# gkv856/speaker_embedding_GE2E_loss

Hardware: AMD Instinct MI355X
Metric: GE2E loss+backward throughput, (spk x utt) batches/sec at N=64 M=10 D=256 (higher is better)
Workload: dtype f32; 1 GPU; cfg2: N=64 M=10 D=256 softmax GE2E fwd+bwd, B=16384 batches per launch per GPU, w=10 b=-5; mode=loss, N=64, M=10, D=256, variant=softmax, batches_per_launch=16384, impl=team, parallelism=dp1 (whole batches per rank, no data-path collective)

## Files before the change

speaker_embedding_ge2e_loss_amd/csrc/ge2e_team_fwd.hip:

```cpp
#include <algorithm>

#include "ge2e_common.hpp"
#include "ge2e_split_gemm.hpp"
#include "ge2e_team.hpp"
#include "ge2e_team_kernel.hpp"
#include "ge2e_team_dev.hpp"

namespace ge2e {

size_t team_fwd_lds_bytes(int rt, int D) {
    return (size_t)2 * rt * D * 2 + (size_t)2 * rt * XP * 4 + (size_t)(2 * rt * 4 + 32 + 16) * sizeof(float);
}

template <int NCH, int MR, int RBT, bool CONTRAST>
__global__ __launch_bounds__(512, 2) void ge2e_team_fwd_kernel(Problem p, TeamKWs L, FusedWs F) {
    extern __shared__ __attribute__((aligned(16))) float smem_f[];
    constexpr int D = 64 * NCH;
    constexpr int P = D;
    const int DG = RBT ? D : p.D;
    const unsigned ROWBG = (unsigned)DG * 4u;
    constexpr TeamKX XO = team_exchange(D);
    constexpr unsigned SC4 = XO.cst[0];
    constexpr int RBC = RBT ? RBT : RBMAX;
    const int RB = RBT ? RBT : L.rt / 16;
    const int RT = 16 * RB;
    const int RBr = RB;
    constexpr bool CT_X = RBT != 0;
    _Float16* const ETh = reinterpret_cast<_Float16*>(smem_f);
    _Float16* const ETl = ETh + RT * P;
    float* const XB0 = reinterpret_cast<float*>(ETl + RT * P);
    float* const XB1 = XB0 + RT * XP;
    float* const RS = XB1 + RT * XP;
    float* const RED = RS + 2 * RT * 4;
    int* const SH = reinterpret_cast<int*>(RED + 32);

    constexpr bool MEX = RBT != 0;
    const int N = MEX ? 64 : p.N, M = MEX ? MR : p.M, NM = N * M;
    const int tid = threadIdx.x;
    const int lane = tid & 63;
    const int wid = __builtin_amdgcn_readfirstlane(tid >> 6);

    TeamCtl* const ctl = reinterpret_cast<TeamCtl*>(p.ws);
    TeamKFlags* const flags = reinterpret_cast<TeamKFlags*>(ctl + 1);
    const TeamId id = team_form(ctl, SH, team_launch_id(p.launch_seq));
    if (id.team == -2) {
        team_redo<NCH>(p, L, F, smem_f, (int)gridDim.x, (int)blockIdx.x);
        __syncthreads();
        if (blockIdx.x == 0 && tid < 64) team_untrusted_done(ctl, (int)(L.head_bytes / 16), team_launch_id(p.launch_seq));
        return;
    }
    if (id.nct == 0 && blockIdx.x == 0 && tid == 0)
        __hip_atomic_store(&ctl->abort_, 1u, __ATOMIC_RELAXED, __HIP_MEMORY_SCOPE_AGENT);
    bool gave_up = id.nct == 0;
    [&]() __attribute__((always_inline)) {
    if (id.team < 0) return;
    TeamKFlags* const fl = flags + id.team;
    const __amdgpu_buffer_rsrc_t rsX = make_rsrc(
        reinterpret_cast<const char*>(p.ws) + L.head_bytes + (size_t)id.team * XO.stride, XO.stride);

    const int spm = MEX ? 8 : L.spm;
    const int w_bits = __builtin_amdgcn_readfirstlane(__float_as_int(p.w ? *p.w : p.w_imm));
    const int b_bits = __builtin_amdgcn_readfirstlane(__float_as_int(p.b ? *p.b : p.b_imm));
    const float eps = p.eps, eps_cos = p.eps_cos;
#define GE2E_TF_CONSTS()                                                                       \
    int wb_ = w_bits, bb_ = b_bits, mc_ = M, le_ = __float_as_int(p.log_eps);                  \
    asm volatile("" : "+s"(wb_), "+s"(bb_), "+s"(mc_), "+s"(le_));                             \
    const float w = __int_as_float(wb_), bias = __int_as_float(bb_);                           \
    const float eps_cos2 = eps_cos * eps_cos;                                                  \
    const float fM = (float)mc_, inv_m = rcp_nr(fM), inv_m1 = rcp_nr((float)(mc_ - 1));       \
    (void)w; (void)bias; (void)eps_cos2; (void)fM; (void)inv_m; (void)inv_m1; (void)le_
    constexpr float LOG2E = 1.4426950408889634f, LN2 = 0.6931471805599453f;

    for (int i = tid; i < RT * P / 8; i += 512) {
        reinterpret_cast<float4*>(ETh)[i] = zero4();
        reinterpret_cast<float4*>(ETl)[i] = zero4();
    }
    for (int i = tid; i < 2 * RT; i += 512) reinterpret_cast<float4*>(RS)[i] = zero4();
    __syncthreads();

    float4 ra[MR], rb2[MR];
    float sn_cur = 0.f, ss_cur = 0.f, sn_prev = 0.f, ss_prev = 0.f;
#define GE2E_TF_LOAD_ROWS(REG, BI)                                                                       \
    do {                                                                                                 \
        int lq_ = lane;                                                                                  \
        asm volatile("" : "+v"(lq_));                                                                    \
        const unsigned vrow_ = 4 * lq_ < DG ? (unsigned)lq_ * 16u : OOB;                                 \
        const bool on_ = has_spk && (BI) < p.B;                                                          \
        const __amdgpu_buffer_rsrc_t rs_ = make_rsrc(p.E + (size_t)(on_ ? (BI) : 0) * NM * DG, (unsigned)NM * ROWBG); \
        _Pragma("unroll") for (int i = 0; i < MR; ++i)                                                   \
            REG[i] = bload4<GE2E_T2_E_AUX>(rs_, (on_ && i < M) ? vrow_ : OOB, (unsigned)(j * M + min(i, M - 1)) * ROWBG); \
    } while (0)
#ifdef GE2E_TF_WITH_PRIO
#define GE2E_TF_PRIO(n) __builtin_amdgcn_s_setprio(n)
#else
#define GE2E_TF_PRIO(n)
#endif
#define GE2E_TF_LOADR_SETUP(BI)                                                                          \
    int lq_ = lane;                                                                                      \
    asm volatile("" : "+v"(lq_));                                                                        \
    const unsigned vrow_ = 4 * lq_ < DG ? (unsigned)lq_ * 16u : OOB;                                     \
    const bool on_ = has_spk && (BI) < p.B;                                                              \
    const __amdgpu_buffer_rsrc_t rs_ = make_rsrc(p.E + (size_t)(on_ ? (BI) : 0) * NM * DG, (unsigned)NM * ROWBG)
#define GE2E_TF_LOADR(REG, I_)                                                                           \
    do {                                                                                                 \
        if ((I_) < MR) {                                                                                 \
            __builtin_amdgcn_sched_barrier(0);                                                           \
            REG[(I_) < MR ? (I_) : 0] = bload4<GE2E_T2_E_AUX>(rs_, (on_ && (I_) < M) ? vrow_ : OOB,      \
                                                              (unsigned)(j * M + min((I_), M - 1)) * ROWBG); \
            __builtin_amdgcn_sched_barrier(0);                                                           \
        }                                                                                                \
    } while (0)
#define GE2E_TF_LANE()                                                  \
    int lv_ = lane;                                                     \
    asm volatile("" : "+v"(lv_));                                       \
    const int l15 = lv_ & 15, q = lv_ >> 4, d4 = 4 * lv_;               \
    const bool dact = D == 256 || d4 < D;                               \
    (void)l15; (void)q; (void)d4; (void)dact

    GE2E_PROF_DECL(20)
    {
        const int j0 = id.member * spm;
        const int my_spm = MEX ? 8 : max(0, min(spm, N - j0));
        const bool has_spk = wid < my_spm;
        const int j = j0 + wid;
        GE2E_TF_LOAD_ROWS(ra, id.team);
        GE2E_TF_LOAD_ROWS(rb2, id.team + id.nct);
    }
    const TeamId id_outer = id;
    bool failed = false;
    int nsig = 0;
    const int wid_outer = wid, member_outer = id.member, tid_outer = tid, m_outer = M;
    float4 sc_pend = zero4();
    int sc_batch = -1;
    auto sc_flush = [&]() __attribute__((always_inline)) {
        if (sc_batch >= 0) {
            const float l = oct_sum(sc_pend.x), a = oct_sum(sc_pend.y), c = oct_sum(sc_pend.z);
            if ((threadIdx.x & 63) == 0) {
                if (p.loss) p.loss[sc_batch] = l;
                if (p.dw) p.dw[sc_batch] = a;
                if (p.db) p.db[sc_batch] = c;
            }
            sc_batch = -1;
        }
    };
    const int nb = id.team < p.B ? (p.B - id.team + id.nct - 1) / id.nct : 0;
    int seq = 0;
    auto body = [&](float4 (&R0)[MR]) __attribute__((always_inline)) {
        int wid_o = wid_outer, mem_o = member_outer, tid_o = tid_outer, m_o = m_outer;
        asm volatile("" : "+s"(wid_o), "+s"(mem_o), "+v"(tid_o), "+s"(m_o));
        const int wid = wid_o, tid = tid_o, lane = tid & 63, M = MEX ? MR : m_o, NM = N * M;
        TeamId id = id_outer;
        id.member = mem_o;
        const int j0 = id.member * spm;
        const int my_spm = MEX ? 8 : max(0, min(spm, N - j0));
        const bool has_spk = wid < my_spm;
        const int j = j0 + wid;
        const int kslot = 8 * id.member + wid;
        const int rbase = wid * M;
        const int tX = wid & 3, khX = wid >> 2;
        const int bi = id.team + seq * id.nct;
        const bool have_cur = seq < nb, have_prev = seq > 0;
        const int buf = seq & 1, pbuf = buf ^ 1;
        sn_prev = sn_cur; ss_prev = ss_cur;

        h8 xa[NCH][2];
        int lx_ = lane;
        asm volatile("" : "+v"(lx_));
        const unsigned oa = have_prev ? XO.chr[pbuf] + ((unsigned)tX * (4u * NCH) + (unsigned)khX * NCH) * 1024u + (unsigned)lx_ * 16u : OOB;
#define GE2E_TF_XA_LOAD(K_)                                                                                        \
    do {                                                                                                           \
        if ((K_) < 2 * NCH) {                                                                                      \
            __builtin_amdgcn_sched_barrier(0);                                                                     \
            xa[((K_) < 2 * NCH ? (K_) : 0) >> 1][(K_) & 1] =                                                       \
                bload_h8<AUX_L2>(rsX, oa + 1024u * (unsigned)((K_) >> 1) + (((K_) & 1) ? 2048u * NCH : 0u), 0);    \
            __builtin_amdgcn_sched_barrier(0);                                                                     \
        }                                                                                                          \
    } while (0)
        if (!have_cur) static_for<0, 2 * NCH>([&](auto kc) { GE2E_TF_XA_LOAD(decltype(kc)::value); });
        if (have_cur) {
            GE2E_TF_LANE();
            GE2E_TF_CONSTS();
            float4 s = zero4();
            static_for<0, MR>([&](auto ic) {
                constexpr int i = decltype(ic)::value;
                if (i < M) { s.x += R0[i].x; s.y += R0[i].y; s.z += R0[i].z; s.w += R0[i].w; }
                GE2E_TF_XA_LOAD(i);
            });
            const float4 c = scale4(s, inv_m);
            float sqs[2] = {dot4(c, c), dot4(s, s)};
            wave_sum_to_sgpr<2>(sqs);
            float rn, kap, nc;
            unit_stats_bf(sqs[0], eps_cos, eps_cos2, rn, kap, nc);
            if (!has_spk) { rn = 0.f; nc = 0.f; }
            sn_cur = has_spk ? fM * nc : 0.f;
            ss_cur = has_spk ? sqs[1] : 0.f;
            h4 hi, lo;
            split4_scaled(c, rn * kSplitScale, hi, lo);
            const unsigned blk = (unsigned)(kslot >> 4) * (4u * NCH) + (unsigned)(lv_ >> 3);
            const unsigned vh = dact ? blk * 1024u + (unsigned)(((lv_ >> 1) & 3) * 16 + (kslot & 15)) * 16u + (unsigned)(lv_ & 1) * 8u : OOB;
            __builtin_amdgcn_raw_buffer_store_b64(__builtin_bit_cast(u32x2, hi), rsX, vh + XO.chr[buf], 0, 0);
            __builtin_amdgcn_raw_buffer_store_b64(__builtin_bit_cast(u32x2, lo), rsX, vh + XO.chr[buf] + 2048u * NCH, 0, 0);
        }
        GE2E_PROF(0);
        GE2E_TF_PRIO(1);

        auto phase_x = [&]() __attribute__((always_inline)) {
        if (have_prev) {
            GE2E_TF_LANE();
            float* const XBk = khX ? XB1 : XB0;
            const int fx = (4 * (l15 & 3) + ((4 - (l15 >> 2)) & 3)) & ((D % 128 == 0) ? 15 : 7);
            h8 fb[2][2];
            f32x4 acc[2] = {acc_zero4(), acc_zero4()};
            int xs[NCH];
#pragma unroll
            for (int s2 = 0; s2 < NCH; ++s2) xs[s2] = l15 * P + (((4 * (khX * NCH + s2) + q) ^ fx) << 3);
#define TF_X_LOAD(T_)                                                                                     \
    do {                                                                                                  \
        const _Float16* const pp_ = ETh + xs[(T_) % NCH] + 16 * ((T_) / NCH) * P;                         \
        fb[(T_) & 1][0] = frag_row(pp_);                                                                  \
        fb[(T_) & 1][1] = frag_row(pp_ + RT * P);                                                         \
    } while (0)
#define TF_X_STORE(RB_)                                                                       \
    *reinterpret_cast<float4*>(XBk + (16 * (RB_) + l15) * XP + 16 * tX + 4 * q) =             \
        make_float4(acc[(RB_) & 1][0], acc[(RB_) & 1][1], acc[(RB_) & 1][2], acc[(RB_) & 1][3])
            TF_X_LOAD(0);
#pragma unroll
            for (int rb = 0; rb < RBC; ++rb) {
                if (CT_X || rb < RBr) {
                    acc[rb & 1] = acc_zero4();
#pragma unroll
                    for (int s = 0; s < NCH; ++s) {
                        const int t = rb * NCH + s;
                        if (t + 1 < RBC * NCH && (CT_X || t + 1 < RBr * NCH)) TF_X_LOAD(t + 1);
                        mfma16x3(acc[rb & 1], xa[s][0], xa[s][1], fb[t & 1][0], fb[t & 1][1]);
                        __builtin_amdgcn_sched_barrier(0);
                    }
                    if (rb > 0) { TF_X_STORE(rb - 1); }
                }
            }
            if (CT_X) { TF_X_STORE(RBT - 1); }
            else {
#pragma unroll
                for (int rb = 0; rb < RBC; ++rb)
                    if (rb == RBr - 1) { TF_X_STORE(rb); }
            }
#undef TF_X_LOAD
#undef TF_X_STORE
        }
        };
        phase_x();
        sc_flush();
        GE2E_PROF(1);

        asm volatile("s_waitcnt vmcnt(0)" ::: "memory");
        GE2E_PROF(2);
        __syncthreads();
        if (tid == 0) add_agent(&fl->c1, 1u);
        ++nsig;
        GE2E_PROF(3);
        GE2E_TF_PRIO(3);

        h4 hiv[MR], lov[MR];
        auto phase_a2c = [&]() __attribute__((always_inline)) {
        if (have_cur && has_spk) {
            GE2E_TF_LANE();
            GE2E_TF_CONSTS();
            float eev[MR];
#pragma unroll
            for (int i = 0; i < MR; ++i) eev[i] = i < M ? dot4(R0[i], R0[i]) : 0.f;
            const float ee_l = wave_sums_scatter<MR>(eev, lv_);
            float rne_l, ke_l, ne_l;
            unit_stats_bf(ee_l, eps_cos, eps_cos2, rne_l, ke_l, ne_l);
            {
                const int rho = lv_ >> 4, irow = 4 * (lv_ & 15) + (((rho & 1) << 1) | (rho >> 1));
                if ((lv_ & 15) < (MR + 3) / 4 && irow < M)
                    *reinterpret_cast<float4*>(RS + (buf * RT + rbase + irow) * 4) = make_float4(rne_l, ke_l, ee_l, ne_l);
            }
            const float rs_l = rne_l * kSplitScale;
            float scv[MR];
#pragma unroll
            for (int i = 0; i < MR; ++i) scv[i] = lane_get(rs_l, scatter_lane(i));
#pragma unroll
            for (int i = 0; i < MR; ++i)
                if (i < M) split4_scaled_hi_u(R0[i], scv[i], hiv[i]);
#pragma unroll
            for (int i = 0; i < MR; ++i)
                if (i < M) split4_scaled_lo_u(R0[i], scv[i], hiv[i], lov[i]);
        }
        };
        phase_a2c();
        if (have_cur && has_spk) {
            GE2E_TF_LANE();
#pragma unroll
            for (int i = 0; i < MR; ++i)
                if (i < M && dact) {
                    const int eo = et_off<D>(rbase + i, d4);
                    *reinterpret_cast<h4*>(ETh + eo) = hiv[i];
                    *reinterpret_cast<h4*>(ETl + eo) = lov[i];
                }
        }
        const bool spread_loads = have_prev && has_spk;
        if (!spread_loads) GE2E_TF_LOAD_ROWS(R0, bi + 2 * id.nct);
        GE2E_PROF(4);
        GE2E_TF_PRIO(1);

        float loss_acc = 0.f, dw_acc = 0.f, db_acc = 0.f;
        if (have_prev && has_spk) {
            GE2E_TF_LANE();
            GE2E_TF_CONSTS();
            const float w2 = w * LOG2E, b2 = (w * eps + bias) * LOG2E, leps2 = __int_as_float(le_) * LOG2E;
            const int rr = lv_ >> 2, qq = lv_ & 3;
            const bool rv = rr < M;
            const int r = rbase + min(rr, M - 1);
            const int ko = kslot;
            const int sb = (ko & ~3) + 16 * qq;
            const int jo = ko & 3;
            const bool own_lane = qq == 0;
            const bool all_valid = N == NC;
            const bool want_wb = p.dw != nullptr || p.db != nullptr;
            GE2E_TF_LOADR_SETUP(bi + 2 * id.nct);
            float x[16];
            float4 xa4[4], xb4[4];
#pragma unroll
            for (int jj = 0; jj < 4; ++jj) {
                const int s4 = (sb + 4 * jj) & (NC - 1);
                xa4[jj] = *reinterpret_cast<const float4*>(XB0 + r * XP + s4);
                xb4[jj] = *reinterpret_cast<const float4*>(XB1 + r * XP + s4);
            }
            GE2E_TF_LOADR(R0, 0);
#pragma unroll
            for (int jj = 0; jj < 4; ++jj) {
                const float4 a = xa4[jj], b = xb4[jj];
                x[4 * jj + 0] = a.x + b.x; x[4 * jj + 1] = a.y + b.y; x[4 * jj + 2] = a.z + b.z; x[4 * jj + 3] = a.w + b.w;
                if (jj == 1) GE2E_TF_LOADR(R0, 1);
            }
            GE2E_TF_LOADR(R0, 2);
            const float xo = (XB0[r * XP + ko] + XB1[r * XP + ko]) * kSplitInv2;
            const float4 rs0 = *reinterpret_cast<const float4*>(RS + (pbuf * RT + r) * 4);
            const float rne = rs0.x, ee = rs0.z, ne = rs0.w;
            const float es = xo * sn_prev * ne;
            const float eu = (es - ee) * inv_m1;
            const float uu = fmaxf((ss_prev - 2.0f * es + ee) * (inv_m1 * inv_m1), 0.0f);
            float rnu, ku, nu;
            unit_stats_bf(uu, eps_cos, eps_cos2, rnu, ku, nu);
            const float cosd = eu * rne * rnu;
            GE2E_TF_LOADR(R0, 3);
            const float sjj2 = fmaf(w2, cosd, b2);
            const float w2s = w2 * kSplitInv2;
            auto vld = [&](int jx) {
                const int s = (sb + jx) & (NC - 1);
                return all_valid || (s & 7) < max(0, min(spm, N - (s >> 3) * spm));
            };
            bool ownj[4];
#pragma unroll
            for (int jx = 0; jx < 4; ++jx) ownj[jx] = own_lane && jo == jx;
            float per, coefsum = 0.f, db_row = 0.f;
            GE2E_TF_PRIO(0);
            GE2E_TF_LOADR(R0, 4);
            if (!CONTRAST) {
                float xm0 = ownj[0] ? x[1] : x[0], xm1 = ownj[1] ? x[0] : x[1], xm2 = ownj[2] ? x[3] : x[2], xm3 = ownj[3] ? x[2] : x[3];
                float xm;
                if (w2 >= 0.f) {
                    xm = fmaxf(fmaxf(xm0, xm1), fmaxf(xm2, xm3));
#pragma unroll
                    for (int jx = 4; jx < 16; jx += 2) xm = fmaxf(fmaxf(x[jx], x[jx + 1]), xm);
                } else {
                    xm = fminf(fminf(xm0, xm1), fminf(xm2, xm3));
#pragma unroll
                    for (int jx = 4; jx < 16; jx += 2) xm = fminf(fminf(x[jx], x[jx + 1]), xm);
                }
                GE2E_TF_LOADR(R0, 5);
                float mx = quad_max(fmaf(w2s, xm, b2));
                mx = fmaxf(fmaxf(mx, sjj2), leps2);
                const float t = b2 - mx;
                float gv[16];
#pragma unroll
                for (int jx = 0; jx < 16; ++jx) {
                    gv[jx] = __builtin_amdgcn_exp2f(fmaf(w2s, x[jx], t));
                    if ((jx & 3) == 3) GE2E_TF_LOADR(R0, 6 + (jx >> 2));
                }
                static_for<10, MR>([&](auto ic) { GE2E_TF_LOADR(R0, decltype(ic)::value); });
                if (!all_valid) {
#pragma unroll
                    for (int jx = 0; jx < 16; ++jx) gv[jx] = vld(jx) ? gv[jx] : 0.f;
                }
#pragma unroll
                for (int jx = 0; jx < 4; ++jx) gv[jx] = ownj[jx] ? 0.f : gv[jx];
                float z4[4] = {gv[0], gv[1], gv[2], gv[3]}, a4[4] = {0.f, 0.f, 0.f, 0.f};
#pragma unroll
                for (int jx = 4; jx < 16; ++jx) z4[jx & 3] += gv[jx];
                const float zl = (z4[0] + z4[1]) + (z4[2] + z4[3]);
                float al = 0.f;
                if (want_wb) {
#pragma unroll
                    for (int jx = 0; jx < 16; ++jx) a4[jx & 3] = fmaf(gv[jx], x[jx], a4[jx & 3]);
                    al = (a4[0] + a4[1]) + (a4[2] + a4[3]);
                }
                const float zp = quad_sum(zl);
                const float zoff = zp + __builtin_amdgcn_exp2f(leps2 - mx);
                const float z = zoff + __builtin_amdgcn_exp2f(sjj2 - mx);
                per = LN2 * ((mx - sjj2) + __builtin_amdgcn_logf(z));
                if (want_wb) {
                    const float ap = quad_sum(al);
                    const float rz = rcp_nr(z);
                    const float ad0 = -zoff * rz;
                    coefsum = fmaf(ap * kSplitInv2, rz, ad0 * cosd);
                    db_row = fmaf(zp, rz, ad0);
                }
            } else {
                static_for<5, MR>([&](auto ic) { GE2E_TF_LOADR(R0, decltype(ic)::value); });
                float best = -INFINITY, bx = 0.f; int besti = 0x7fffffff;
#pragma unroll
                for (int jx = 0; jx < 16; ++jx) {
                    const int s = (sb + jx) & (NC - 1);
                    const bool ok = vld(jx) && !(jx < 4 && ownj[jx & 3]);
                    const float sve = ok ? fmaf(w2s, x[jx], b2) : -INFINITY;
                    if (ok && (sve > best || (sve == best && s < besti))) { best = sve; besti = s; bx = x[jx]; }
                }
                const int loci = besti;
                quad_argmax(best, besti);
                bx = quad_sum(loci == besti && besti != 0x7fffffff ? bx : 0.f);
                const float pos = rcp_nr(1.0f + __builtin_amdgcn_exp2f(-sjj2));
                const float neg = (N > 1) ? rcp_nr(1.0f + __builtin_amdgcn_exp2f(-best)) : 0.0f;
                per = 1.0f - pos + neg;
                const float ad0 = -pos * (1.0f - pos);
                const float gn = neg * (1.0f - neg);
                coefsum = fmaf(gn, bx * kSplitInv2, ad0 * cosd);
                db_row = gn + ad0;
            }
            if (rv && own_lane) {
                loss_acc = per;
                dw_acc = fmaf(eps, db_row, coefsum);
                db_acc = db_row;
                if (p.per) p.per[(size_t)(bi - id.nct) * NM + j0 * M + rbase + rr] = per;
            }
        }
        __builtin_amdgcn_sched_barrier(0);
        if (have_prev) {
            if (p.dw != nullptr || p.db != nullptr) {
                float v3[3] = {loss_acc, dw_acc, db_acc};
                wave_sum_to_sgpr<3>(v3);
                if (lane == 0) { RED[wid] = v3[0]; RED[8 + wid] = v3[1]; RED[16 + wid] = v3[2]; }
            } else {
                float v1[1] = {loss_acc};
                wave_sum_to_sgpr<1>(v1);
                if (lane == 0) { RED[wid] = v1[0]; RED[8 + wid] = 0.f; RED[16 + wid] = 0.f; }
            }
        }
        GE2E_PROF(5);

        {
            int* const wsh = SH + 4 + (seq & 3);
            if (tid == 0) *wsh = spin_until(&fl->c1, (unsigned)(TEAM * nsig), ctl) ? 1 : 0;
            __syncthreads();
            failed = *wsh == 0;
        }
        GE2E_PROF(6);
        GE2E_TF_PRIO(3);

        if (have_prev && tid == 0) {
            float l = 0.f, a = 0.f, c = 0.f;
#pragma unroll
            for (int i = 0; i < 8; ++i) { l += RED[i]; a += RED[8 + i]; c += RED[16 + i]; }
            bstore4(rsX, SC4 + (unsigned)((seq - 1) & 3) * 128u + (unsigned)id.member * 16u, make_float4(l, a, c, 0.f));
        }
        if (seq >= 2 && id.member == 0 && wid == 0) {
            GE2E_TF_LANE();
            sc_pend = bload4<AUX_L2>(rsX, lv_ < TEAM ? SC4 + (unsigned)((seq - 2) & 3) * 128u + (unsigned)lv_ * 16u : OOB, 0);
            sc_batch = bi - 2 * id.nct;
        }
        GE2E_PROF(7);
        GE2E_TF_PRIO(2);
        ++seq;
    };
    if (nb > 0) for (;;) {
        body(ra);
        if (seq > nb || failed) break;
        body(rb2);
        if (seq > nb || failed) break;
    }
    if (!failed) sc_flush();
    if (!failed) {
        int mem_o = member_outer, tid_o = tid_outer;
        asm volatile("" : "+s"(mem_o), "+v"(tid_o));
        const int tid = tid_o, lane = tid & 63;
        if (nb > 0) {
            asm volatile("s_waitcnt vmcnt(0)" ::: "memory");
            __syncthreads();
            if (tid == 0) add_agent(&fl->c1, 1u);
            ++nsig;
            if (mem_o == 0 && tid < 64) {
                int okv = 1;
                if (lane == 0) okv = spin_until(&fl->c1, (unsigned)(TEAM * nsig), ctl) ? 1 : 0;
                if (__builtin_amdgcn_readfirstlane(okv) != 0) {
                    const int first = nb >= 2 ? nb - 1 : 0;
                    for (int k = first; k < nb; ++k) {
                        const float4 scv = bload4<AUX_L2>(rsX, lane < TEAM ? SC4 + (unsigned)(k & 3) * 128u + (unsigned)lane * 16u : OOB, 0);
                        const float l = oct_sum(scv.x), a = oct_sum(scv.y), c = oct_sum(scv.z);
                        if (lane == 0) {
                            const int bo = id.team + k * id.nct;
                            if (p.loss) p.loss[bo] = l;
                            if (p.dw) p.dw[bo] = a;
                            if (p.db) p.db[bo] = c;
                        }
                    }
                } else {
                    failed = true;
                }
            }
        }
    }
    if (failed && (threadIdx.x & 63) == 0) __hip_atomic_store(&ctl->abort_, 1u, __ATOMIC_RELAXED, __HIP_MEMORY_SCOPE_AGENT);
    gave_up = gave_up || failed;
    GE2E_PROF_FLUSH(20)
    }();
    {
        if (p.test_abort == 2 && blockIdx.x == (gridDim.x >> 1)) {
            if (threadIdx.x == 0) __hip_atomic_store(&ctl->abort_, 1u, __ATOMIC_RELAXED, __HIP_MEMORY_SCOPE_AGENT);
            gave_up = true;
        }
        int* const fsh = reinterpret_cast<int*>(smem_f) + 4;
        const TeamRedo rd = team_finish(ctl, fsh, (int)(L.head_bytes / 16), gave_up);
        if (rd.n != 0) {
            team_redo<NCH>(p, L, F, smem_f, rd.n, rd.rank);
            team_redo_done(ctl, fsh, (int)(L.head_bytes / 16), rd.n);
        }
    }
#undef GE2E_TF_LOAD_ROWS
#undef GE2E_TF_LANE
#undef GE2E_TF_CONSTS
}

template <int NCH, int MR, int RBT, bool CONTRAST>
static hipError_t launch_fwd_nch(Problem& p, TeamKWs& L, const FusedWs& F, hipStream_t stream) {
    const void* fn = reinterpret_cast<const void*>(ge2e_team_fwd_kernel<NCH, MR, RBT, CONTRAST>);
    static KernelLaunchState state;
    unsigned lds = (unsigned)team_fwd_lds_bytes(L.rt, 64 * NCH);
    lds = std::max(lds, (unsigned)fused_split_lds_bytes(p.D));
    int nb = 0;
    hipError_t err = prepare_kernel(state, fn, 512, lds, &nb);
    if (err != hipSuccess) return err;
    if (p.test_abort == 1) {
        err = launch_team_head_init(p.ws, L.head_bytes, true, stream);
        if (err != hipSuccess) return err;
    }
    int grid = team_grid(p.B);
    if (p.grid_cap > 0 && p.grid_cap < grid)
        grid = p.grid_cap / (MAX_XCD * TEAM) * (MAX_XCD * TEAM) > 0 ? p.grid_cap / (MAX_XCD * TEAM) * (MAX_XCD * TEAM) : MAX_XCD * TEAM;
    if (nb < 1 || grid > nb * device_cu_count()) return hipErrorCooperativeLaunchTooLarge;
    hipLaunchKernelGGL((ge2e_team_fwd_kernel<NCH, MR, RBT, CONTRAST>), dim3(grid), dim3(512), lds, stream, p, L, F);
    return hipGetLastError();
}
template <int NCH, int MR>
static hipError_t launch_fwd_variant(Problem& p, TeamKWs& L, const FusedWs& F, const TeamPlan& plan, hipStream_t stream) {
    if (NCH == 4 && MR == 10 && plan.rbt == 5)
        return plan.contrast ? launch_fwd_nch<4, 10, 5, true>(p, L, F, stream) : launch_fwd_nch<4, 10, 5, false>(p, L, F, stream);
    return plan.contrast ? launch_fwd_nch<NCH, MR, 0, true>(p, L, F, stream) : launch_fwd_nch<NCH, MR, 0, false>(p, L, F, stream);
}

hipError_t launch_team_fwd(Problem& p, TeamKWs& L, const FusedWs& F, hipStream_t stream) {
    const TeamPlan plan = plan_team(p.N, p.M, p.D, p.variant);
    switch (plan.mr * 10 + plan.nch) {
        case 101: return launch_fwd_variant<1, 10>(p, L, F, plan, stream);
        case 102: return launch_fwd_variant<2, 10>(p, L, F, plan, stream);
        case 103: return launch_fwd_variant<3, 10>(p, L, F, plan, stream);
        case 104: return launch_fwd_variant<4, 10>(p, L, F, plan, stream);
        case 161: return launch_fwd_variant<1, 16>(p, L, F, plan, stream);
        case 162: return launch_fwd_variant<2, 16>(p, L, F, plan, stream);
        case 163: return launch_fwd_variant<3, 16>(p, L, F, plan, stream);
        default: return launch_fwd_variant<4, 16>(p, L, F, plan, stream);
    }
}

}
```

Baseline: 2.253 million batches/s.

## Interleave centroid phase into X-phase MFMA loop with s-outer ordering and prefetched xa

Restructures the team forward kernel so the centroid/normalisation phase (A1) for the current batch is split into slices and interleaved between the MFMAs of the previous batch's X-phase GEMM. It also reorders the X-phase loop to iterate the K-chunk on the outside with one accumulator per row block, and prefetches the first xa fragments at the end of the previous iteration. The aim is to hide A1's ALU work, its reduction latency and the global xa load latency behind matrix-core work. The cost is higher register pressure from more accumulators and more complex scheduling under sched_barrier constraints.

```diff
diff --git a/speaker_embedding_ge2e_loss_amd/csrc/ge2e_team_fwd.hip b/speaker_embedding_ge2e_loss_amd/csrc/ge2e_team_fwd.hip
--- a/speaker_embedding_ge2e_loss_amd/csrc/ge2e_team_fwd.hip
+++ b/speaker_embedding_ge2e_loss_amd/csrc/ge2e_team_fwd.hip
@@ -26,6 +26,8 @@
     const int RT = 16 * RB;
     const int RBr = RB;
     constexpr bool CT_X = RBT != 0;
+    constexpr bool S_OUTER = RBT != 0 || MR <= 10;
+    constexpr bool MERGE = S_OUTER;
     _Float16* const ETh = reinterpret_cast<_Float16*>(smem_f);
     _Float16* const ETl = ETh + RT * P;
     float* const XB0 = reinterpret_cast<float*>(ETl + RT * P);
@@ -90,6 +92,9 @@
         _Pragma("unroll") for (int i = 0; i < MR; ++i)                                                   \
             REG[i] = bload4<GE2E_T2_E_AUX>(rs_, (on_ && i < M) ? vrow_ : OOB, (unsigned)(j * M + min(i, M - 1)) * ROWBG); \
     } while (0)
+#ifndef GE2E_TF_A1_STRIDE
+#define GE2E_TF_A1_STRIDE 3
+#endif
 #ifdef GE2E_TF_WITH_PRIO
 #define GE2E_TF_PRIO(n) __builtin_amdgcn_s_setprio(n)
 #else
@@ -132,6 +137,7 @@
     const int wid_outer = wid, member_outer = id.member, tid_outer = tid, m_outer = M;
     float4 sc_pend = zero4();
     int sc_batch = -1;
+    h8 xa_lead[2] = {};
     auto sc_flush = [&]() __attribute__((always_inline)) {
         if (sc_batch >= 0) {
             const float l = oct_sum(sc_pend.x), a = oct_sum(sc_pend.y), c = oct_sum(sc_pend.z);
@@ -164,91 +170,158 @@
         sn_prev = sn_cur; ss_prev = ss_cur;
 
         h8 xa[NCH][2];
+        constexpr int XA0 = S_OUTER ? 2 : 0;
+        if constexpr (S_OUTER) { xa[0][0] = xa_lead[0]; xa[0][1] = xa_lead[1]; }
         int lx_ = lane;
         asm volatile("" : "+v"(lx_));
         const unsigned oa = have_prev ? XO.chr[pbuf] + ((unsigned)tX * (4u * NCH) + (unsigned)khX * NCH) * 1024u + (unsigned)lx_ * 16u : OOB;
 #define GE2E_TF_XA_LOAD(K_)                                                                                        \
     do {                                                                                                           \
-        if ((K_) < 2 * NCH) {                                                                                      \
-            __builtin_amdgcn_sched_barrier(0);                                                                     \
+        if ((K_) >= XA0 && (K_) < 2 * NCH)                                                                         \
             xa[((K_) < 2 * NCH ? (K_) : 0) >> 1][(K_) & 1] =                                                       \
                 bload_h8<AUX_L2>(rsX, oa + 1024u * (unsigned)((K_) >> 1) + (((K_) & 1) ? 2048u * NCH : 0u), 0);    \
-            __builtin_amdgcn_sched_barrier(0);                                                                     \
-        }                                                                                                          \
     } while (0)
-        if (!have_cur) static_for<0, 2 * NCH>([&](auto kc) { GE2E_TF_XA_LOAD(decltype(kc)::value); });
-        if (have_cur) {
+        {
             GE2E_TF_LANE();
             GE2E_TF_CONSTS();
-            float4 s = zero4();
-            static_for<0, MR>([&](auto ic) {
-                constexpr int i = decltype(ic)::value;
-                if (i < M) { s.x += R0[i].x; s.y += R0[i].y; s.z += R0[i].z; s.w += R0[i].w; }
-                GE2E_TF_XA_LOAD(i);
-            });
-            const float4 c = scale4(s, inv_m);
-            float sqs[2] = {dot4(c, c), dot4(s, s)};
-            wave_sum_to_sgpr<2>(sqs);
-            float rn, kap, nc;
-            unit_stats_bf(sqs[0], eps_cos, eps_cos2, rn, kap, nc);
-            if (!has_spk) { rn = 0.f; nc = 0.f; }
-            sn_cur = has_spk ? fM * nc : 0.f;
-            ss_cur = has_spk ? sqs[1] : 0.f;
-            h4 hi, lo;
-            split4_scaled(c, rn * kSplitScale, hi, lo);
-            const unsigned blk = (unsigned)(kslot >> 4) * (4u * NCH) + (unsigned)(lv_ >> 3);
-            const unsigned vh = dact ? blk * 1024u + (unsigned)(((lv_ >> 1) & 3) * 16 + (kslot & 15)) * 16u + (unsigned)(lv_ & 1) * 8u : OOB;
-            __builtin_amdgcn_raw_buffer_store_b64(__builtin_bit_cast(u32x2, hi), rsX, vh + XO.chr[buf], 0, 0);
-            __builtin_amdgcn_raw_buffer_store_b64(__builtin_bit_cast(u32x2, lo), rsX, vh + XO.chr[buf] + 2048u * NCH, 0, 0);
-        }
-        GE2E_PROF(0);
-        GE2E_TF_PRIO(1);
-
-        auto phase_x = [&]() __attribute__((always_inline)) {
-        if (have_prev) {
-            GE2E_TF_LANE();
-            float* const XBk = khX ? XB1 : XB0;
-            const int fx = (4 * (l15 & 3) + ((4 - (l15 >> 2)) & 3)) & ((D % 128 == 0) ? 15 : 7);
-            h8 fb[2][2];
-            f32x4 acc[2] = {acc_zero4(), acc_zero4()};
-            int xs[NCH];
-#pragma unroll
-            for (int s2 = 0; s2 < NCH; ++s2) xs[s2] = l15 * P + (((4 * (khX * NCH + s2) + q) ^ fx) << 3);
-#define TF_X_LOAD(T_)                                                                                     \
-    do {                                                                                                  \
-        const _Float16* const pp_ = ETh + xs[(T_) % NCH] + 16 * ((T_) / NCH) * P;                         \
-        fb[(T_) & 1][0] = frag_row(pp_);                                                                  \
-        fb[(T_) & 1][1] = frag_row(pp_ + RT * P);                                                         \
-    } while (0)
+            constexpr int A1N = MR + 7;
+            constexpr int A1G = GE2E_TF_A1_STRIDE;
+            float4 a1s = zero4(), a1c = zero4();
+            float a1q[2] = {0.f, 0.f};
+            float a1rn = 0.f;
+            h4 a1hi = {}, a1lo = {};
+            auto a1_slice = [&](auto kc, auto with_loads) __attribute__((always_inline)) {
+                constexpr int k = decltype(kc)::value;
+                if constexpr (decltype(with_loads)::value) GE2E_TF_XA_LOAD(k + XA0);
+                if constexpr (k < MR) {
+                    if (k < M) { a1s.x += R0[k].x; a1s.y += R0[k].y; a1s.z += R0[k].z; a1s.w += R0[k].w; }
+                } else if constexpr (k == MR) {
+                    a1c = scale4(a1s, inv_m);
+                } else if constexpr (k == MR + 1) {
+                    a1q[0] = dot4(a1c, a1c);
+                } else if constexpr (k == MR + 2) {
+                    a1q[1] = dot4(a1s, a1s);
+                } else if constexpr (k == MR + 3) {
+                    wave_sum_to_sgpr<2>(a1q);
+                } else if constexpr (k == MR + 4) {
+                    float rn, kap, nc;
+                    unit_stats_bf(a1q[0], eps_cos, eps_cos2, rn, kap, nc);
+                    if (!has_spk) { rn = 0.f; nc = 0.f; }
+                    sn_cur = has_spk ? fM * nc : 0.f;
+                    ss_cur = has_spk ? a1q[1] : 0.f;
+                    a1rn = rn;
+                } else if constexpr (k == MR + 5) {
+                    split4_scaled(a1c, a1rn * kSplitScale, a1hi, a1lo);
+                } else if constexpr (k == MR + 6) {
+                    const unsigned blk = (unsigned)(kslot >> 4) * (4u * NCH) + (unsigned)(lv_ >> 3);
+                    const unsigned vh = dact ? blk * 1024u + (unsigned)(((lv_ >> 1) & 3) * 16 + (kslot & 15)) * 16u + (unsigned)(lv_ & 1) * 8u : OOB;
+                    __builtin_amdgcn_raw_buffer_store_b64(__builtin_bit_cast(u32x2, a1hi), rsX, vh + XO.chr[buf], 0, 0);
+                    __builtin_amdgcn_raw_buffer_store_b64(__builtin_bit_cast(u32x2, a1lo), rsX, vh + XO.chr[buf] + 2048u * NCH, 0, 0);
+                }
+            };
+            if (have_cur && (!MERGE || !have_prev))
+                static_for<0, A1N>([&](auto kc) {
+                    a1_slice(kc, std::integral_constant<bool, !MERGE>{});
+                    __builtin_amdgcn_sched_barrier(0);
+                });
+            GE2E_PROF(0);
+            GE2E_TF_PRIO(1);
+
+            auto x_run = [&](auto with_a1) __attribute__((always_inline)) {
+                constexpr bool WA = decltype(with_a1)::value;
+                float* const XBk = khX ? XB1 : XB0;
+                const int fx = (4 * (l15 & 3) + ((4 - (l15 >> 2)) & 3)) & ((D % 128 == 0) ? 15 : 7);
+                int xs[NCH];
+#pragma unroll
+                for (int s2 = 0; s2 < NCH; ++s2) xs[s2] = l15 * P + (((4 * (khX * NCH + s2) + q) ^ fx) << 3);
+                constexpr int NACC = S_OUTER ? RBC : 2;
+                f32x4 acc[NACC];
+#pragma unroll
+                for (int a = 0; a < NACC; ++a) acc[a] = acc_zero4();
+                auto frag = [&](int off, h8 (&f)[2]) __attribute__((always_inline)) {
+                    const _Float16* const pp = ETh + off;
+                    f[0] = frag_row(pp);
+                    f[1] = frag_row(pp + RT * P);
+                };
+#define TF_X_ACC(RB_) acc[S_OUTER ? (RB_) : (RB_) & 1]
 #define TF_X_STORE(RB_)                                                                       \
     *reinterpret_cast<float4*>(XBk + (16 * (RB_) + l15) * XP + 16 * tX + 4 * q) =             \
-        make_float4(acc[(RB_) & 1][0], acc[(RB_) & 1][1], acc[(RB_) & 1][2], acc[(RB_) & 1][3])
-            TF_X_LOAD(0);
-#pragma unroll
-            for (int rb = 0; rb < RBC; ++rb) {
-                if (CT_X || rb < RBr) {
-                    acc[rb & 1] = acc_zero4();
-#pragma unroll
-                    for (int s = 0; s < NCH; ++s) {
-                        const int t = rb * NCH + s;
-                        if (t + 1 < RBC * NCH && (CT_X || t + 1 < RBr * NCH)) TF_X_LOAD(t + 1);
-                        mfma16x3(acc[rb & 1], xa[s][0], xa[s][1], fb[t & 1][0], fb[t & 1][1]);
-                        __builtin_amdgcn_sched_barrier(0);
+        make_float4(TF_X_ACC(RB_)[0], TF_X_ACC(RB_)[1], TF_X_ACC(RB_)[2], TF_X_ACC(RB_)[3])
+#define TF_X_MFMA(A_, B_, FIRST_)                                                             \
+    do {                                                                                      \
+        __builtin_amdgcn_sched_barrier(0);                                                    \
+        asm volatile("" ::"v"(cin));                                                          \
+        if constexpr (!(FIRST_)) cin = TF_X_ACC(rb);       \
+        mfma16(TF_X_ACC(rb), A_, B_);                                                         \
+    } while (0)
+#define TF_X_FILL(I_)                                                                         \
+    do {                                                                                      \
+        if constexpr (WA && (3 * t + (I_)) % A1G == 0 && (3 * t + (I_)) / A1G < A1N) {        \
+            __builtin_amdgcn_sched_barrier(0);                                                \
+            a1_slice(std::integral_constant<int, (3 * t + (I_)) / A1G>{}, std::true_type{});  \
+            asm volatile("" ::"v"(fc[0]), "v"(fc[1]), "v"(xa[s][0]), "v"(xa[s][1]));          \
+            __builtin_amdgcn_sched_barrier(0);                                                \
+        }                                                                                     \
+    } while (0)
+                h8 fc[2], fn[2];
+                f32x4 cin = acc_zero4();
+                if constexpr (WA) { a1s = zero4(); a1c = zero4(); a1q[0] = 0.f; a1q[1] = 0.f; a1rn = 0.f; }
+                frag(xs[0], fn);
+                static_for<0, NCH * RBC>([&](auto tc) {
+                    constexpr int t = decltype(tc)::value;
+                    constexpr int s = S_OUTER ? t / RBC : t % NCH, rb = S_OUTER ? t % RBC : t / NCH;
+                    if (CT_X || rb < RBr) {
+                        fc[0] = fn[0];
+                        fc[1] = fn[1];
+                        if constexpr (!S_OUTER) {
+                            if constexpr (s == 0) TF_X_ACC(rb) = acc_zero4();
+                            if constexpr (t + 1 < RBC * NCH) {
+                                if (t + 1 < RBr * NCH) frag(xs[(t + 1) % NCH] + 16 * ((t + 1) / NCH) * P, fn);
+                            }
+                        } else if constexpr (rb + 1 < RBC) {
+                            if constexpr (CT_X) frag(xs[s] + 16 * (rb + 1) * P, fn);
+                            else if constexpr (s + 1 < NCH) frag(rb + 1 < RBr ? xs[s] + 16 * (rb + 1) * P : xs[s + 1 < NCH ? s + 1 : s], fn);
+                            else { if (rb + 1 < RBr) frag(xs[s] + 16 * (rb + 1) * P, fn); }
+                        } else if constexpr (s + 1 < NCH) {
+                            frag(xs[s + 1 < NCH ? s + 1 : s], fn);
+                        }
+                        TF_X_MFMA(xa[s][0], fc[0], S_OUTER && s == 0);
                     }
-                    if (rb > 0) { TF_X_STORE(rb - 1); }
-                }
-            }
-            if (CT_X) { TF_X_STORE(RBT - 1); }
-            else {
-#pragma unroll
-                for (int rb = 0; rb < RBC; ++rb)
-                    if (rb == RBr - 1) { TF_X_STORE(rb); }
-            }
-#undef TF_X_LOAD
+                    TF_X_FILL(0);
+                    if (CT_X || rb < RBr) TF_X_MFMA(xa[s][0], fc[1], false);
+                    TF_X_FILL(1);
+                    if (CT_X || rb < RBr) {
+                        TF_X_MFMA(xa[s][1], fc[0], false);
+                        if constexpr (S_OUTER && s == NCH - 1 && rb > 0) { TF_X_STORE(rb > 0 ? rb - 1 : 0); }
+                        if constexpr (!S_OUTER && s == 0 && rb > 0) { TF_X_STORE(rb > 0 ? rb - 1 : 0); }
+                    }
+                    TF_X_FILL(2);
+                    __builtin_amdgcn_sched_barrier(0);
+                });
+                if constexpr (WA) static_for<(3 * NCH * RBC + A1G - 1) / A1G, A1N>([&](auto kc) { a1_slice(kc, std::true_type{}); });
+                if (CT_X) { TF_X_STORE(RBC - 1); }
+                else {
+#pragma unroll
+                    for (int rb = 0; rb < RBC; ++rb)
+                        if (rb == RBr - 1) { TF_X_STORE(rb); }
+                }
+                __builtin_amdgcn_sched_barrier(0);
+                asm volatile("" ::"v"(cin));
+#undef TF_X_MFMA
+#undef TF_X_FILL
+#undef TF_X_ACC
 #undef TF_X_STORE
-        }
-        };
-        phase_x();
+            };
+            if (have_prev) {
+                if (MERGE && have_cur) {
+                    x_run(std::integral_constant<bool, MERGE>{});
+                } else {
+                    if (!have_cur) static_for<XA0, 2 * NCH>([&](auto kc) { GE2E_TF_XA_LOAD(decltype(kc)::value); });
+                    x_run(std::false_type{});
+                }
+            }
+        }
+#undef GE2E_TF_XA_LOAD
         sc_flush();
         GE2E_PROF(1);
 
@@ -458,6 +531,13 @@
         GE2E_PROF(6);
         GE2E_TF_PRIO(3);
 
+        if constexpr (S_OUTER) {
+            int ln_ = lane;
+            asm volatile("" : "+v"(ln_));
+            const unsigned on = have_cur ? XO.chr[buf] + ((unsigned)tX * (4u * NCH) + (unsigned)khX * NCH) * 1024u + (unsigned)ln_ * 16u : OOB;
+            xa_lead[0] = bload_h8<AUX_L2>(rsX, on, 0);
+            xa_lead[1] = bload_h8<AUX_L2>(rsX, on + 2048u * NCH, 0);
+        }
         if (have_prev && tid == 0) {
             float l = 0.f, a = 0.f, c = 0.f;
 #pragma unroll
```

Result: no change. 2.258 million batches/s, median of 3 (+0.2%).
